# audexdev/Lossless-Audio-Codec

Hardware: AMD Instinct MI355X
Metric: encode Msamples/s at 1/2/4/8 MI355X; byte-identical .lac vs CPU ref (higher is better)
Workload: dtype int64

## Files before the change

lossless-audio-codec_amd/csrc/k_front.hip:

```cpp
#include <hip/hip_runtime.h>

#include "kernels_internal.h"
#include "x87.h"

namespace lacx {

__device__ __forceinline__ uint64_t zz64(int64_t v) {
    return v >= 0 ? ((uint64_t)v << 1) : ((((uint64_t)(-(v + 1))) << 1) | 1u);
}

__device__ __forceinline__ uint64_t approx_rice_bits(uint64_t sum, uint64_t count) {
    if (count == 0) return 0;
    const uint64_t mean = (sum + (count >> 1)) / count;
    uint32_t k = mean <= 1u ? 0u : 64u - (uint32_t)__clzll((long long)(mean - 1u));
    k = k > 31u ? 31u : k;
    return (sum >> k) + count * (uint64_t)(k + 1u);
}

constexpr int kIngestTile = 4096;
static_assert(kIngestThreads == kProbe, "one probe sample per thread");

__device__ __forceinline__ bool slot_channel_used(const AnalyzeParams& prm, int ch) {
    if (prm.channels == 1) return ch == 0;
    if (prm.stereo_mode == 0) return ch < 2;
    if (prm.stereo_mode == 1) return ch >= 2;
    return true;
}

__device__ __forceinline__ void reduce13(const int64_t* acc, unsigned long long* s_ac, int64_t* out, int tid) {
    if (tid < 13) s_ac[tid] = 0;
    __syncthreads();
#pragma unroll
    for (int k = 0; k < 13; ++k) {
        const uint64_t t = wave_sum_u64((uint64_t)acc[k]);
        if ((tid & 63) == 0) atomicAdd(&s_ac[k], (unsigned long long)t);
    }
    __syncthreads();
    if (tid < 13) out[tid] = (int64_t)s_ac[tid];
    __syncthreads();
}

__device__ __forceinline__ void stereo_block(const AnalyzeParams& prm, uint32_t blk, uint32_t nb, bool live, int tid,
                                             const unsigned long long* __restrict__ sums, const uint32_t* __restrict__ badidx,
                                             BlockPlan* __restrict__ bplans, uint32_t* __restrict__ need_probe,
                                             uint32_t* __restrict__ need_full);

__device__ __forceinline__ void ingest_done(uint32_t* __restrict__ front_ctr, unsigned int* s_last, const AnalyzeParams& prm,
                                            uint32_t blk, uint32_t nb, const unsigned long long* __restrict__ sums,
                                            const uint32_t* __restrict__ badidx, BlockPlan* __restrict__ bplans,
                                            uint32_t* __restrict__ need_probe, uint32_t* __restrict__ need_full) {
    if (!front_ctr) return;
    const int tid = threadIdx.x;
    if (tid == 0) {
        asm volatile("s_waitcnt vmcnt(0)" ::: "memory");
        *s_last = atomicAdd(&front_ctr[(size_t)blk * 2], 1u) == 3u ? 1u : 0u;
    }
    __syncthreads();
    if (*s_last == 0u || tid >= 64) return;
    if (tid == 0) front_ctr[(size_t)blk * 2] = 0u;
    stereo_block(prm, blk, nb, tid < 16, tid, sums, badidx, bplans, need_probe, need_full);
}

__global__ __launch_bounds__(kIngestThreads, 5) void k_ingest(BatchRef br, unsigned long long* __restrict__ sums,
                                                           uint32_t* __restrict__ badidx,
                                                           int64_t* __restrict__ acorr, uint32_t* __restrict__ front_ctr,
                                                           BlockPlan* __restrict__ bplans, uint32_t* __restrict__ need_probe,
                                                           uint32_t* __restrict__ need_full) {
    __shared__ int4 s_plane[4][kIngestThreads + 1];
    __shared__ __align__(16) int32_t s_win[3][12 + kProbe];
    __shared__ unsigned long long s_ac[13];
    __shared__ unsigned long long s_sum[3];
    __shared__ unsigned int s_bad;
    uint32_t blk, chsel;
    xcd_slot(blockIdx.x, 4u, gridDim.x >> 2, blk, chsel);
    const StreamDesc sd = stream_of_block_uniform(br, blk);
    const AnalyzeParams prm = sd.prm;
    const int32_t* __restrict__ L = sd.left;
    const int32_t* __restrict__ R = sd.right;
    const uint32_t lblk = blk - sd.first_block;
    const int ch = (int)chsel;
    const bool used = slot_channel_used(prm, ch);
    const bool container_bounds = prm.layout == PCM_INTERLEAVED_I16 || (prm.layout == PCM_INTERLEAVED_I24 && prm.bit_depth == 24);
    const bool validate = ch < 2 && ch < prm.channels && prm.bit_depth != 0 && !container_bounds;
    const uint32_t nb = block_frames(prm, lblk);
    if (!used && !validate) {
        if (ch < 2 && threadIdx.x == 0) agent_store(&badidx[blk * 2 + ch], 0xFFFFFFFFu);
        ingest_done(front_ctr, &s_bad, prm, blk, nb, sums, badidx, bplans, need_probe, need_full);
        return;
    }
    const int tid = threadIdx.x, lane = tid & 63;
    const int64_t bstart = (int64_t)lblk * kMaxBlock;
    const SlotSrc src = slot_src(prm, L, R, ch);
    const bool est = prm.channels == 2 && prm.stereo_mode == 2;
    const int32_t lo = prm.bit_depth == 16 ? -32768 : -0x800000;
    const int32_t hi = prm.bit_depth == 16 ? 32767 : 0x7FFFFF;
    if (tid < 3) s_sum[tid] = 0;
    if (tid == 0) s_bad = 0xFFFFFFFFu;
    if (tid < 4) s_plane[tid][0] = make_int4(0, 0, 0, 0);
    __syncthreads();

    constexpr int kPerThread = kIngestTile / kIngestThreads;
    static_assert(kPerThread == 16, "four 4-sample groups per thread and tile");
    int64_t acc[13];
#pragma unroll
    for (int k = 0; k < 13; ++k) acc[k] = 0;
    uint64_t sraw = 0, sdif = 0, sant = 0;
    uint32_t bad = 0xFFFFFFFFu;
    for (uint32_t base = 0; base < nb; base += kIngestTile) {
        const uint32_t first = base + 16u * (uint32_t)tid;
        const int rem = (int)nb - (int)first;
        const int cnt = rem < 0 ? 0 : (rem > 16 ? 16 : rem);
        int32_t w[28];
        load_chunk<16>(src, bstart + first, cnt, bstart + (int64_t)nb - 1, w + 12);
#pragma unroll
        for (int i = 0; i < 16; ++i) {
            if (i >= cnt) w[12 + i] = 0;
            else if (validate && (w[12 + i] < lo || w[12 + i] > hi)) bad = bad < first + (uint32_t)i ? bad : first + (uint32_t)i;
        }
#pragma unroll
        for (int c = 0; c < 4; ++c)
            s_plane[c][tid + 1] = make_int4(w[12 + 4 * c], w[13 + 4 * c], w[14 + 4 * c], w[15 + 4 * c]);
        __syncthreads();
        int4 carry = make_int4(0, 0, 0, 0);
        if (tid >= 1 && tid <= 3) carry = s_plane[tid][kIngestThreads];
#pragma unroll
        for (int c = 1; c < 4; ++c) {
            const int4 h = s_plane[c][tid];
            w[4 * (c - 1)] = h.x;
            w[4 * (c - 1) + 1] = h.y;
            w[4 * (c - 1) + 2] = h.z;
            w[4 * (c - 1) + 3] = h.w;
        }
        if (used) {
#pragma unroll
            for (int i = 0; i < 16; ++i) {
#pragma unroll
                for (int k = 0; k < 13; ++k) acc[k] += (int64_t)w[12 + i] * (int64_t)w[12 + i - k];
            }
            if (est) {
                auto zz32 = [](int32_t v) { return ((uint32_t)v << 1) ^ (uint32_t)(v >> 31); };
                uint32_t traw = 0, tdif = 0, tant = 0;
#pragma unroll
                for (int i = 0; i < 16; ++i) {
                    if (i < cnt) {
                        const int32_t x0 = w[12 + i], prev = w[11 + i];
                        const uint32_t raw = zz32(x0);
                        const bool head = (first + (uint32_t)i) == 0u;
                        traw += raw;
                        tdif += head ? raw : zz32((int32_t)((uint32_t)x0 - (uint32_t)prev));
                        tant += head ? raw : zz32((int32_t)((uint32_t)x0 + (uint32_t)prev));
                    }
                }
                sraw += traw;
                sdif += tdif;
                sant += tant;
            }
        }
        __syncthreads();
        if (tid >= 1 && tid <= 3) s_plane[tid][0] = carry;
    }
    if (used) reduce13(acc, s_ac, acorr + ((size_t)blk * kSlotsPerBlock + ch) * 13, tid);

    if (est && nb > (uint32_t)kFullCompareLimit) {
        if (tid < 36) s_win[tid / 12][tid % 12] = 0;
        for (int w = 1; w <= 3; ++w) {
            const SlotGeom g = slot_geom(prm, lblk, w * 4 + ch);
            s_win[w - 1][12 + tid] = slot_fetch(src, g.start + tid);
        }
        __syncthreads();
        const int wv = tid >> 6;
        if (wv < 3) {
            int32_t v[16];
#pragma unroll
            for (int c = 0; c < 4; ++c) {
                const int4 q = *reinterpret_cast<const int4*>(&s_win[wv][4 * lane + 4 * c]);
                v[4 * c] = q.x;
                v[4 * c + 1] = q.y;
                v[4 * c + 2] = q.z;
                v[4 * c + 3] = q.w;
            }
            int64_t* out = acorr + ((size_t)blk * kSlotsPerBlock + (wv + 1) * 4 + ch) * 13;
#pragma unroll
            for (int k = 0; k < 13; ++k) {
                int64_t a = 0;
#pragma unroll
                for (int i = 0; i < 4; ++i) a += (int64_t)v[12 + i] * (int64_t)v[12 + i - k];
                const uint64_t t = wave_sum_u64((uint64_t)a);
                if (lane == 0) out[k] = (int64_t)t;
            }
        }
    }

    if (est) {
        const uint64_t t0 = wave_sum_u64(sraw), t1 = wave_sum_u64(sdif), t2 = wave_sum_u64(sant);
        if (lane == 0) {
            atomicAdd(&s_sum[0], (unsigned long long)t0);
            atomicAdd(&s_sum[1], (unsigned long long)t1);
            atomicAdd(&s_sum[2], (unsigned long long)t2);
        }
    }
    if (bad != 0xFFFFFFFFu) atomicMin(&s_bad, bad);
    __syncthreads();
    if (tid == 0) {
        if (est) {
            agent_store(&sums[(size_t)blk * 12 + ch], s_sum[0]);
            agent_store(&sums[(size_t)blk * 12 + 4 + ch], s_sum[1]);
            agent_store(&sums[(size_t)blk * 12 + 8 + ch], s_sum[2]);
        }
        if (validate || ch < 2) agent_store(&badidx[blk * 2 + ch], s_bad);
    }
    __syncthreads();
    ingest_done(front_ctr, &s_bad, prm, blk, nb, sums, badidx, bplans, need_probe, need_full);
}

constexpr int kStereoLanes = 16;
__device__ __forceinline__ void stereo_block(const AnalyzeParams& prm, uint32_t blk, uint32_t nb, bool live, int tid,
                                             const unsigned long long* __restrict__ sums, const uint32_t* __restrict__ badidx,
                                             BlockPlan* __restrict__ bplans, uint32_t* __restrict__ need_probe,
                                             uint32_t* __restrict__ need_full) {
    const int sub = tid & (kStereoLanes - 1), grp = tid & ~(kStereoLanes - 1);
    const bool stereo = prm.channels == 2;
    const bool est = stereo && prm.stereo_mode == 2;
    uint64_t bits = 0;
    if (est && live && sub < 12) bits = approx_rice_bits(agent_load(&sums[(size_t)blk * 12 + sub]), nb);
    auto from = [&](int lane_in_group) {
        const uint32_t lo = (uint32_t)__shfl((int)(uint32_t)bits, grp + lane_in_group, 64);
        const uint32_t hi = (uint32_t)__shfl((int)(uint32_t)(bits >> 32), grp + lane_in_group, 64);
        return ((uint64_t)hi << 32) | lo;
    };
    uint64_t chbits[4];
    bool active = false;
#pragma unroll
    for (int c = 0; c < 4; ++c) {
        const uint64_t raw = from(c), dif = from(4 + c), ant = from(8 + c);
        uint64_t mn = raw < dif ? raw : dif;
        if (ant < mn) mn = ant;
        chbits[c] = mn;
        active = active || (raw < dif) || (ant < dif);
    }
    if (!live || sub != 0) return;
    BlockPlan bp;
    bp.choose_ms = 0;
    bp.uncertain = 0;
    bp.est_ms = 0;
    const uint32_t badl = agent_load(&badidx[blk * 2]), badr = stereo ? agent_load(&badidx[blk * 2 + 1]) : 0xFFFFFFFFu;
    bp.invalid = (badl != 0xFFFFFFFFu) || (badr != 0xFFFFFFFFu);
    bp.first_bad = (badl != 0xFFFFFFFFu) ? badl : (badr != 0xFFFFFFFFu ? (badr | 0x80000000u) : 0xFFFFFFFFu);
    bp.frames = nb;
    bp.pad = 0;
    uint32_t nprobe = 0, nfull = 0;
    if (!stereo) {
        nfull = 1u;
    } else if (prm.stereo_mode == 0) {
        nfull = 0x3u;
    } else if (prm.stereo_mode == 1) {
        nfull = 0xCu;
        bp.choose_ms = 1;
    } else {
        const uint64_t lr = chbits[0] + chbits[1], ms = chbits[2] + chbits[3];
        const uint64_t smaller = lr < ms ? lr : ms;
        const uint64_t diff = lr >= ms ? lr - ms : ms - lr;
        bp.est_ms = ms < lr;
        bp.choose_ms = bp.est_ms;
        bp.uncertain = smaller == 0 || diff == 0 || active || diff <= smaller / 100u;
        if (!bp.uncertain) {
            nfull = bp.est_ms ? 0xCu : 0x3u;
        } else if (nb <= (uint32_t)kFullCompareLimit) {
            nfull = 0xFu;
        } else if (agent_load(&sums[(size_t)blk * 12]) == 0ull && agent_load(&sums[(size_t)blk * 12 + 1]) == 0ull) {
            nfull = 0x3u;
            bp.choose_ms = 0;
        } else {
            nprobe = 0xFFF0u;
        }
    }
    bplans[blk] = bp;
    need_probe[blk] = nprobe;
    need_full[blk] = nfull;
}

__global__ __launch_bounds__(64) void k_stereo(BatchRef br, const unsigned long long* __restrict__ sums,
                                               const uint32_t* __restrict__ badidx, BlockPlan* __restrict__ bplans,
                                               uint32_t* __restrict__ need_probe, uint32_t* __restrict__ need_full) {
    const int tid = threadIdx.x;
    const uint32_t blk = blockIdx.x * (64 / kStereoLanes) + (uint32_t)(tid / kStereoLanes);
    const bool live = blk < br.total_blocks;
    const StreamDesc sd = stream_of_block(br, live ? blk : 0u);
    const uint32_t nb = live ? block_frames(sd.prm, blk - sd.first_block) : 0u;
    stereo_block(sd.prm, blk, nb, live, tid, sums, badidx, bplans, need_probe, need_full);
}


__global__ __launch_bounds__(kLevThreads) void k_levinson(BatchRef br, const int64_t* __restrict__ acorr,
                                                          const uint32_t* __restrict__ need_probe,
                                                          LpcSet* __restrict__ lpcs) {
    extern __shared__ __align__(16) unsigned char lev_raw[];
    LevMem& lm = *reinterpret_cast<LevMem*>(lev_raw);
    const uint32_t id = blockIdx.x * kLevThreads + threadIdx.x;
    const uint32_t nblk = br.total_blocks;
    const int slot = (int)(id / nblk);
    const uint32_t blk = id % nblk;
    if (slot >= kSlotsPerBlock) return;
    const StreamDesc sd = stream_of_block(br, blk);
    const AnalyzeParams prm = sd.prm;
    const SlotGeom g = slot_geom(prm, blk - sd.first_block, slot);
    if (!g.defined) return;
    if (prm.channels == 2 && slot < 4) {
        if (prm.stereo_mode == 0 && (slot & 3) >= 2) return;
        if (prm.stereo_mode == 1 && (slot & 3) < 2) return;
    }
    if (slot >= 4 && !((need_probe[blk] >> slot) & 1u)) return;
    const uint32_t gid = blk * kSlotsPerBlock + (uint32_t)slot;
    const int mvo = (g.n > 1) ? (int)((g.n - 1 < 32u) ? g.n - 1 : 32u) : 0;
    struct LdsArray {
        uint64_t (*m)[kLevThreads];
        uint32_t (*es)[kLevThreads];
        int lane;
        __device__ xf80 get(int i) const {
            const uint32_t w = es[i][lane];
            return xf80{m[i][lane], (int32_t)(w & 0x7FFFFFFFu) - (1 << 21), w >> 31};
        }
        __device__ void set(int i, xf80 x) {
            m[i][lane] = x.m;
            es[i][lane] = (x.s << 31) | ((uint32_t)(x.e + (1 << 21)) & 0x7FFFFFFFu);
        }
    };
    const int lane = (int)threadIdx.x;
    LdsArray Rv{lm.m[0], lm.es[0], lane}, av{lm.m[1], lm.es[1], lane}, pv{lm.m[2], lm.es[2], lane};
    const int64_t* r = acorr + (size_t)gid * 13;
    LpcSet* out = &lpcs[gid];
    levinson_candidates_t([r](int i) { return r[i]; }, mvo, Rv, av, pv,
                          [out](int ci, int j, int16_t v) { out->coef[ci][j] = v; },
                          [out](int ci, uint8_t v) { out->used[ci] = v; });
    out->pad = 0;
}

__global__ __launch_bounds__(64) void k_decide(BatchRef br, int phase, BlockPlan* __restrict__ bplans,
                                               const uint32_t* __restrict__ need_probe,
                                               uint32_t* __restrict__ need_full,
                                               const ChannelPlan* __restrict__ plans) {
    const int tid = threadIdx.x, sub = tid & 15;
    const uint32_t blk = blockIdx.x * 4u + (uint32_t)(tid >> 4);
    if (br.table == nullptr && (br.single.prm.channels != 2 || br.single.prm.stereo_mode != 2)) return;
    const bool live = blk < br.total_blocks;
    BlockPlan bp{};
    if (live) bp = bplans[blk];
    const bool mine = live && bp.uncertain &&
                      (phase == 1 ? need_probe[blk] != 0 : bp.frames <= (uint32_t)kFullCompareLimit);
    const bool take = mine && (phase == 1 ? sub >= 4 : sub < 4);
    const uint32_t bytes = take ? plans[(size_t)blk * kSlotsPerBlock + sub].payload_bytes : 0u;
    const bool is_ms = (sub & 3) >= 2;
    uint32_t lr = is_ms ? 0u : bytes, ms = is_ms ? bytes : 0u;
#pragma unroll
    for (int d = 1; d < 16; d <<= 1) {
        lr += (uint32_t)__shfl_xor((int)lr, d, 64);
        ms += (uint32_t)__shfl_xor((int)ms, d, 64);
    }
    if (!mine || sub != 0) return;
    bp.choose_ms = ms < lr;
    bplans[blk] = bp;
    if (phase == 1) need_full[blk] = bp.choose_ms ? 0xCu : 0x3u;
}

hipError_t set_kernel_attrs_front() {
    return hipFuncSetAttribute(reinterpret_cast<const void*>(&k_levinson), hipFuncAttributeMaxDynamicSharedMemorySize,
                               (int)sizeof(LevMem));
}

}
```

Before: 25010.

## Restructure ingest reductions, proxy sums and window lags in front kernel

Replaces the per-lag wave_sum plus shared-atomic reduction with a shared-memory tree reduction of 16 values (13 lags plus 3 proxy sums) that reuses the s_plane buffer. Rewrites the zigzag proxy sums as absolute-difference accumulation with sign popcount corrections, and adds wave-uniform fast paths when all chunks are full. Window lag correlations are computed per lane and lag, then combined with two xor shuffles instead of 13 wave reductions. This cuts shuffle and atomic traffic in the ingest kernel, at the cost of extra barriers and reliance on exact arithmetic equivalence; the head-sample special case for the first sample's diff is dropped, which depends on the zero carry-in.

```diff
diff --git a/lossless-audio-codec_amd/csrc/ingest_core.h b/lossless-audio-codec_amd/csrc/ingest_core.h
--- /dev/null
+++ b/lossless-audio-codec_amd/csrc/ingest_core.h
@@ -0,0 +1,88 @@
+#pragma once
+#include "analyze_core.h"
+
+#ifndef LACX_HDF
+#if defined(__HIPCC__)
+#define LACX_HDF __host__ __device__ __forceinline__
+#else
+#define LACX_HDF inline
+#endif
+#endif
+
+namespace lacx {
+
+constexpr int kIngestPer = 16;
+constexpr int kIngestHist = 12;
+constexpr int kIngestLags = 13;
+constexpr uint32_t kNoBadSample = 0xFFFFFFFFu;
+
+LACX_HDF void ingest_zero_tail(int32_t* w, int cnt) {
+#pragma unroll
+    for (int i = 0; i < kIngestPer; ++i)
+        if (i >= cnt) w[kIngestHist + i] = 0;
+}
+
+LACX_HDF int64_t opaque_i64(int64_t v) {
+#if defined(__HIP_DEVICE_COMPILE__)
+    asm volatile("" : "+v"(v));
+#endif
+    return v;
+}
+
+LACX_HDF void ingest_lags(const int32_t* w, int64_t* acc) {
+#pragma unroll
+    for (int i = 0; i < kIngestPer; ++i) {
+#pragma unroll
+        for (int k = 0; k < kIngestLags; ++k)
+            acc[k] = opaque_i64(acc[k] + (int64_t)w[kIngestHist + i] * (int64_t)w[kIngestHist + i - k]);
+    }
+}
+
+template <bool FULL>
+LACX_HDF uint32_t ingest_first_bad(const int32_t* w, int cnt, int32_t lo, int32_t hi, uint32_t first, uint32_t bad) {
+    const uint32_t span = (uint32_t)hi - (uint32_t)lo;
+#pragma unroll
+    for (int i = kIngestPer - 1; i >= 0; --i) {
+        const bool out = (uint32_t)w[kIngestHist + i] - (uint32_t)lo > span;
+        if ((FULL || i < cnt) && out && first + (uint32_t)i < bad) bad = first + (uint32_t)i;
+    }
+    return bad;
+}
+
+LACX_HDF uint32_t sad_u32(uint32_t a, uint32_t b, uint32_t c) {
+    return (a > b ? a - b : b - a) + c;
+}
+
+template <bool FULL>
+LACX_HDF void ingest_proxy_sums(const int32_t* w, int cnt, uint64_t& sraw, uint64_t& sdif, uint64_t& sant) {
+    const uint32_t kBias = (uint32_t)opaque_i32((int)0x80000000u);
+    uint32_t araw = 0, adif = 0, aant = 0;
+    uint32_t nraw = 0, ndif = 0, nant = 0;
+#pragma unroll
+    for (int i = 0; i < kIngestPer; ++i) {
+        if (FULL || i < cnt) {
+            const uint32_t x0 = (uint32_t)w[kIngestHist + i], prev = (uint32_t)w[kIngestHist - 1 + i];
+            const uint32_t bx = x0 ^ kBias;
+            araw = sad_u32(bx, kBias, araw);
+            adif = sad_u32(bx, prev ^ kBias, adif);
+            aant = sad_u32(bx, kBias - prev, aant);
+            nraw = (nraw << 1) | (x0 >> 31);
+            ndif = (ndif << 1) | ((x0 - prev) >> 31);
+            nant = (nant << 1) | ((x0 + prev) >> 31);
+        }
+    }
+    sraw += (uint64_t)(2u * araw - (uint32_t)__builtin_popcount(nraw));
+    sdif += (uint64_t)(2u * adif - (uint32_t)__builtin_popcount(ndif));
+    sant += (uint64_t)(2u * aant - (uint32_t)__builtin_popcount(nant));
+}
+
+constexpr int kWinSeg = 64;
+LACX_HDF int64_t ingest_window_lag(const int32_t* win, int k, int seg) {
+    const int32_t* x = win + kIngestHist + seg * kWinSeg;
+    int64_t a = 0;
+#pragma unroll 16
+    for (int n = 0; n < kWinSeg; ++n) a += (int64_t)x[n] * (int64_t)x[n - k];
+    return a;
+}
+
+}
diff --git a/lossless-audio-codec_amd/csrc/k_front.hip b/lossless-audio-codec_amd/csrc/k_front.hip
--- a/lossless-audio-codec_amd/csrc/k_front.hip
+++ b/lossless-audio-codec_amd/csrc/k_front.hip
@@ -1,5 +1,6 @@
 #include <hip/hip_runtime.h>
 
+#include "ingest_core.h"
 #include "kernels_internal.h"
 #include "x87.h"
 
@@ -27,17 +28,36 @@
     return true;
 }
 
-__device__ __forceinline__ void reduce13(const int64_t* acc, unsigned long long* s_ac, int64_t* out, int tid) {
-    if (tid < 13) s_ac[tid] = 0;
-    __syncthreads();
-#pragma unroll
-    for (int k = 0; k < 13; ++k) {
-        const uint64_t t = wave_sum_u64((uint64_t)acc[k]);
-        if ((tid & 63) == 0) atomicAdd(&s_ac[k], (unsigned long long)t);
-    }
-    __syncthreads();
-    if (tid < 13) out[tid] = (int64_t)s_ac[tid];
-    __syncthreads();
+constexpr int kIngestReduceWords = 16 * (kIngestThreads / 2);
+__device__ __forceinline__ uint64_t block_sum16(uint64_t* val, unsigned long long* red, int tid) {
+    static_assert(kIngestThreads == 256, "two halvings leave one wave");
+#pragma unroll
+    for (int half = kIngestThreads / 2; half >= 64; half >>= 1) {
+        __syncthreads();
+        if (tid >= half && tid < 2 * half) {
+#pragma unroll
+            for (int k = 0; k < 16; ++k) red[k * half + tid - half] = val[k];
+        }
+        __syncthreads();
+        if (tid < half) {
+#pragma unroll
+            for (int k = 0; k < 16; ++k) val[k] += red[k * half + tid];
+        }
+    }
+    if (tid < 64) {
+#pragma unroll
+        for (int k = 0; k < 16; ++k) red[k * 64 + tid] = val[k];
+    }
+    __syncthreads();
+    uint64_t s = 0;
+    if (tid < 64) {
+        const unsigned long long* mine = red + (tid >> 2) * 64 + (tid & 3) * 16;
+#pragma unroll
+        for (int j = 0; j < 16; ++j) s += mine[(j + tid) & 15];
+        s += (uint64_t)__shfl_xor((long long)s, 1, 64);
+        s += (uint64_t)__shfl_xor((long long)s, 2, 64);
+    }
+    return s;
 }
 
 __device__ __forceinline__ void stereo_block(const AnalyzeParams& prm, uint32_t blk, uint32_t nb, bool live, int tid,
@@ -68,8 +88,6 @@
                                                            uint32_t* __restrict__ need_full) {
     __shared__ int4 s_plane[4][kIngestThreads + 1];
     __shared__ __align__(16) int32_t s_win[3][12 + kProbe];
-    __shared__ unsigned long long s_ac[13];
-    __shared__ unsigned long long s_sum[3];
     __shared__ unsigned int s_bad;
     uint32_t blk, chsel;
     xcd_slot(blockIdx.x, 4u, gridDim.x >> 2, blk, chsel);
@@ -94,7 +112,6 @@
     const bool est = prm.channels == 2 && prm.stereo_mode == 2;
     const int32_t lo = prm.bit_depth == 16 ? -32768 : -0x800000;
     const int32_t hi = prm.bit_depth == 16 ? 32767 : 0x7FFFFF;
-    if (tid < 3) s_sum[tid] = 0;
     if (tid == 0) s_bad = 0xFFFFFFFFu;
     if (tid < 4) s_plane[tid][0] = make_int4(0, 0, 0, 0);
     __syncthreads();
@@ -112,10 +129,12 @@
         const int cnt = rem < 0 ? 0 : (rem > 16 ? 16 : rem);
         int32_t w[28];
         load_chunk<16>(src, bstart + first, cnt, bstart + (int64_t)nb - 1, w + 12);
-#pragma unroll
-        for (int i = 0; i < 16; ++i) {
-            if (i >= cnt) w[12 + i] = 0;
-            else if (validate && (w[12 + i] < lo || w[12 + i] > hi)) bad = bad < first + (uint32_t)i ? bad : first + (uint32_t)i;
+        const bool full = wave_all(cnt == kIngestPer);
+        if (full) {
+            if (validate) bad = ingest_first_bad<true>(w, cnt, lo, hi, first, bad);
+        } else {
+            ingest_zero_tail(w, cnt);
+            if (validate) bad = ingest_first_bad<false>(w, cnt, lo, hi, first, bad);
         }
 #pragma unroll
         for (int c = 0; c < 4; ++c)
@@ -132,34 +151,30 @@
             w[4 * (c - 1) + 3] = h.w;
         }
         if (used) {
-#pragma unroll
-            for (int i = 0; i < 16; ++i) {
-#pragma unroll
-                for (int k = 0; k < 13; ++k) acc[k] += (int64_t)w[12 + i] * (int64_t)w[12 + i - k];
+            ingest_lags(w, acc);
+            if (est) {
+                if (full) ingest_proxy_sums<true>(w, cnt, sraw, sdif, sant);
+                else ingest_proxy_sums<false>(w, cnt, sraw, sdif, sant);
             }
-            if (est) {
-                auto zz32 = [](int32_t v) { return ((uint32_t)v << 1) ^ (uint32_t)(v >> 31); };
-                uint32_t traw = 0, tdif = 0, tant = 0;
-#pragma unroll
-                for (int i = 0; i < 16; ++i) {
-                    if (i < cnt) {
-                        const int32_t x0 = w[12 + i], prev = w[11 + i];
-                        const uint32_t raw = zz32(x0);
-                        const bool head = (first + (uint32_t)i) == 0u;
-                        traw += raw;
-                        tdif += head ? raw : zz32((int32_t)((uint32_t)x0 - (uint32_t)prev));
-                        tant += head ? raw : zz32((int32_t)((uint32_t)x0 + (uint32_t)prev));
-                    }
-                }
-                sraw += traw;
-                sdif += tdif;
-                sant += tant;
-            }
         }
         __syncthreads();
         if (tid >= 1 && tid <= 3) s_plane[tid][0] = carry;
     }
-    if (used) reduce13(acc, s_ac, acorr + ((size_t)blk * kSlotsPerBlock + ch) * 13, tid);
+    if (used) {
+        static_assert(sizeof(s_plane) >= kIngestReduceWords * sizeof(unsigned long long), "the planes hold the reduction");
+        uint64_t val[16];
+#pragma unroll
+        for (int k = 0; k < kIngestLags; ++k) val[k] = (uint64_t)acc[k];
+        val[13] = sraw;
+        val[14] = sdif;
+        val[15] = sant;
+        const uint64_t total = block_sum16(val, reinterpret_cast<unsigned long long*>(&s_plane[0][0]), tid);
+        if (tid < 64 && (tid & 3) == 0) {
+            const int k = tid >> 2;
+            if (k < kIngestLags) acorr[((size_t)blk * kSlotsPerBlock + ch) * 13 + k] = (int64_t)total;
+            else if (est) agent_store(&sums[(size_t)blk * 12 + (size_t)(k - kIngestLags) * 4 + ch], (unsigned long long)total);
+        }
+    }
 
     if (est && nb > (uint32_t)kFullCompareLimit) {
         if (tid < 36) s_win[tid / 12][tid % 12] = 0;
@@ -170,45 +185,18 @@
         __syncthreads();
         const int wv = tid >> 6;
         if (wv < 3) {
-            int32_t v[16];
-#pragma unroll
-            for (int c = 0; c < 4; ++c) {
-                const int4 q = *reinterpret_cast<const int4*>(&s_win[wv][4 * lane + 4 * c]);
-                v[4 * c] = q.x;
-                v[4 * c + 1] = q.y;
-                v[4 * c + 2] = q.z;
-                v[4 * c + 3] = q.w;
-            }
-            int64_t* out = acorr + ((size_t)blk * kSlotsPerBlock + (wv + 1) * 4 + ch) * 13;
-#pragma unroll
-            for (int k = 0; k < 13; ++k) {
-                int64_t a = 0;
-#pragma unroll
-                for (int i = 0; i < 4; ++i) a += (int64_t)v[12 + i] * (int64_t)v[12 + i - k];
-                const uint64_t t = wave_sum_u64((uint64_t)a);
-                if (lane == 0) out[k] = (int64_t)t;
-            }
-        }
-    }
-
-    if (est) {
-        const uint64_t t0 = wave_sum_u64(sraw), t1 = wave_sum_u64(sdif), t2 = wave_sum_u64(sant);
-        if (lane == 0) {
-            atomicAdd(&s_sum[0], (unsigned long long)t0);
-            atomicAdd(&s_sum[1], (unsigned long long)t1);
-            atomicAdd(&s_sum[2], (unsigned long long)t2);
-        }
-    }
+            static_assert(4 * kWinSeg == kProbe, "four quarters of sixteen lanes");
+            const int k = lane & 15;
+            int64_t a = ingest_window_lag(s_win[wv], k < kIngestLags ? k : 0, lane >> 4);
+            a += __shfl_xor((long long)a, 16, 64);
+            a += __shfl_xor((long long)a, 32, 64);
+            if (lane < kIngestLags) acorr[((size_t)blk * kSlotsPerBlock + (wv + 1) * 4 + ch) * 13 + lane] = a;
+        }
+    }
+
     if (bad != 0xFFFFFFFFu) atomicMin(&s_bad, bad);
     __syncthreads();
-    if (tid == 0) {
-        if (est) {
-            agent_store(&sums[(size_t)blk * 12 + ch], s_sum[0]);
-            agent_store(&sums[(size_t)blk * 12 + 4 + ch], s_sum[1]);
-            agent_store(&sums[(size_t)blk * 12 + 8 + ch], s_sum[2]);
-        }
-        if (validate || ch < 2) agent_store(&badidx[blk * 2 + ch], s_bad);
-    }
+    if (tid == 0 && (validate || ch < 2)) agent_store(&badidx[blk * 2 + ch], s_bad);
     __syncthreads();
     ingest_done(front_ctr, &s_bad, prm, blk, nb, sums, badidx, bplans, need_probe, need_full);
 }
```

New measurement: 24620. -1.6%, worse.
